# Christovis/astrild

Measured on AMD Instinct MI355X. Metric: particles/sec CIC+3D-FFT P(k) on 1024^3 grid, higher is better.
Workload: dtype f32

## Files before the change

### astrild_amd/csrc/mesh_paint_tiled.hip

```cpp
#include "ast_common.h"
#include "paint_tile_geom.h"
#include <algorithm>
#include <climits>
#include <cstdlib>
#include <mutex>
#include <type_traits>
#include <vector>

namespace {

using ast::Window;

using ast::TX;
using ast::TY;
using ast::TZ;
using ast::RingMap;
#ifndef PAINT_ABLATE
#define PAINT_ABLATE 0
#endif
constexpr int ablate = PAINT_ABLATE;

#ifdef PAINT_STAMPS
__device__ unsigned long long g_stamps[64 * 4096];
__device__ unsigned g_nstamp[64];
#define STAMP_DECL unsigned nst_ = 0
#define STAMP(id)                                                                                     \
    do {                                                                                              \
        if (threadIdx.x == 0 && blockIdx.x % 257 == 3 && blockIdx.x / 257 < 64 && nst_ < 4096)         \
            g_stamps[(blockIdx.x / 257) * 4096 + nst_++] = (__builtin_amdgcn_s_memtime() << 8) | (id); \
    } while (0)
#define STAMP_END                                                                                     \
    do {                                                                                              \
        if (threadIdx.x == 0 && blockIdx.x % 257 == 3 && blockIdx.x / 257 < 64) g_nstamp[blockIdx.x / 257] = nst_; \
    } while (0)
#else
#define STAMP_DECL
#define STAMP(id) do {} while (0)
#define STAMP_END do {} while (0)
#endif
#if defined(PAINT_STAMPS) && PAINT_STAMPS == 2
#define FSTAMP_DECL STAMP_DECL
#define FSTAMP(id) STAMP(id)
#define FSTAMP_END STAMP_END
#define DSTAMP_DECL
#define DSTAMP(id) do {} while (0)
#define DSTAMP_END do {} while (0)
#else
#define FSTAMP_DECL
#define FSTAMP(id) do {} while (0)
#define FSTAMP_END do {} while (0)
#define DSTAMP_DECL STAMP_DECL
#define DSTAMP(id) STAMP(id)
#define DSTAMP_END STAMP_END
#endif

struct TileGeom {
    int n, x_start, nx_alloc;
    int ntx, nty, ntz;
    double inv_dx;
    double shift;
    int off_lo, off_hi;
};

template <typename T> __device__ inline double grid_coord(T x, const TileGeom& g) { return __fma_rn((double)x, g.inv_dx, g.shift); }

template <typename T, int W, bool PLAINX>
__device__ inline uint32_t tile_of(T x, T y, T z, const TileGeom& g, uint32_t* __restrict__ col_flags) {
    const double sx = grid_coord(x, g), sy = grid_coord(y, g), sz = grid_coord(z, g);
    int cx = (int)floor(W == 2 ? sx : sx + 0.5);
    int cy = (int)floor(W == 2 ? sy : sy + 0.5);
    int cz = (int)floor(W == 2 ? sz : sz + 0.5);
    const bool far = max(max((unsigned)cx, (unsigned)cy), (unsigned)cz) >= (unsigned)g.n;
    if (far) {
        double f;
        cx = ast::locate<W>(sx, g.n, f);
        cy = ast::locate<W>(sy, g.n, f);
        cz = ast::locate<W>(sz, g.n, f);
    }
    unsigned bx = (unsigned)cx;
    if (!PLAINX) {
        int b = cx - g.x_start;
        if (b < 0) b += g.n;
        if (b >= g.nx_alloc) return 0xffffffffu;
        bx = (unsigned)b;
    }
    const uint32_t col = __umul24(bx / TX, (unsigned)g.nty) + (unsigned)cy / TY;
    if (far && col_flags && !(__hip_atomic_load(&col_flags[col], __ATOMIC_RELAXED, __HIP_MEMORY_SCOPE_AGENT) & 1u))
        atomicOr(&col_flags[col], 1u);
    return __umul24(col, (unsigned)g.ntz) + (unsigned)cz / TZ;
}

struct WaveRuns {
    bool head;
    int len;
    int head_lane;
};

__device__ inline WaveRuns wave_runs(uint32_t key, bool live, int lane) {
    WaveRuns r;
    const uint32_t prev = (uint32_t)__builtin_amdgcn_update_dpp((int)0xffffffffu, (int)key, 0x138, 0xf, 0xf, false);
    r.head = live && (lane == 0 || prev != key);
    const unsigned long long hmask = __ballot(r.head);
    const unsigned long long dmask = __ballot(!live);
    const unsigned long long above = ~((2ull << lane) - 1ull);
    const unsigned long long stop = (hmask | dmask) & above;
    const int end = stop ? __ffsll((long long)stop) - 1 : 64;
    r.len = end - lane;
    const unsigned long long at_or_below = hmask & ~above;
    r.head_lane = at_or_below ? 63 - __clzll((long long)at_or_below) : 0;
    return r;
}

constexpr int IDX_UNROLL = 4;
#ifndef AGG_TRIPS_N
#define AGG_TRIPS_N 4
#endif
constexpr int AGG_TRIPS = AGG_TRIPS_N;
constexpr int AGG_SLOTS = 256;
constexpr uint32_t SLOT_EMPTY = 0xffffffffu;
constexpr uint32_t CODE_DONE = 0xffffffffu;

template <int MODE>
__device__ __noinline__ void place_run_slow(uint32_t key, uint32_t p1, uint32_t len, const uint32_t* __restrict__ tile_off,
                                            uint32_t* __restrict__ tile_fill, uint32_t* __restrict__ index, uint32_t cap,
                                            uint32_t* __restrict__ ovf, unsigned long long* __restrict__ ovf_count) {
    const uint32_t b = atomicAdd(&tile_fill[key], len);
    for (uint32_t i = 0; i < len; ++i) {
        if (MODE == 1) index[(size_t)tile_off[key] + b + i] = p1 + i;
        else if (b + i < cap) index[(size_t)key * cap + b + i] = p1 + i;
        else ovf[atomicAdd(ovf_count, 1ull)] = p1 + i;
    }
}

template <typename T, int W, int MODE, bool PLAINX, int STRIDE = 3>
__global__ void __launch_bounds__(256)
tile_index_kernel(const T* __restrict__ pos, size_t np, TileGeom g, uint32_t* __restrict__ tile_count,
                  const uint32_t* __restrict__ tile_off, uint32_t* __restrict__ tile_fill,
                  uint32_t* __restrict__ index, uint32_t cap, uint32_t* __restrict__ ovf,
                  unsigned long long* __restrict__ ovf_count, uint32_t* __restrict__ col_flags,
                  unsigned long long* dropped, const unsigned long long* __restrict__ np_dev = nullptr,
                  unsigned long long np_min = 0) {
    constexpr bool FILL = MODE != 0;
    if (np_dev != nullptr) {
        const unsigned long long nd = *np_dev;
        if (nd < np_min || nd == 0) return;
        np = nd < np ? (size_t)nd : np;
    }
    __shared__ uint32_t skey[AGG_SLOTS], scnt[AGG_SLOTS], sroom[AGG_SLOTS];
    __shared__ unsigned long long sdst[AGG_SLOTS];
    __shared__ uint32_t codes[FILL ? AGG_TRIPS * IDX_UNROLL : 1][256];
    constexpr uint32_t MISS_CAP = FILL ? 512 : 1;
    __shared__ uint32_t smiss_key[MISS_CAP], smiss_p[MISS_CAP], smiss_len[MISS_CAP], smiss_n;
    FSTAMP_DECL;
    const int tid = threadIdx.x;
    const int lane = tid & 63;
    skey[tid] = SLOT_EMPTY;
    scnt[tid] = 0;
    if (tid == 0) smiss_n = 0;
    __syncthreads();
    const size_t per_trip = 256 * IDX_UNROLL;
    const size_t per_interval = per_trip * AGG_TRIPS;
    const size_t nintervals = (np + per_interval - 1) / per_interval;
    unsigned long long ndrop = 0;
    auto fetch = [&](size_t pbase, T (&x)[IDX_UNROLL], T (&y)[IDX_UNROLL], T (&z)[IDX_UNROLL]) {
#pragma unroll
        for (int u = 0; u < IDX_UNROLL; ++u) {
            const size_t p = min(pbase + (size_t)u * 256 + tid, np - 1);
            x[u] = pos[STRIDE * p + 0];
            y[u] = pos[STRIDE * p + 1];
            z[u] = pos[STRIDE * p + 2];
        }
    };
    auto place_run = [&](uint32_t key, uint32_t p1, uint32_t len) {
        place_run_slow<MODE>(key, p1, len, tile_off, tile_fill, index, cap, ovf, ovf_count);
    };
    static_assert(AGG_TRIPS % 2 == 0, "two register sets");
    T xa[IDX_UNROLL], ya[IDX_UNROLL], za[IDX_UNROLL], xb[IDX_UNROLL], yb[IDX_UNROLL], zb[IDX_UNROLL];
    if ((size_t)blockIdx.x < nintervals) fetch((size_t)blockIdx.x * per_interval, xa, ya, za);
    for (size_t interval = blockIdx.x; interval < nintervals; interval += gridDim.x) {
        const size_t p0 = interval * per_interval;
        const bool full = p0 + per_interval <= np;
        auto process = [&](int trip, const T (&x)[IDX_UNROLL], const T (&y)[IDX_UNROLL], const T (&z)[IDX_UNROLL]) {
#pragma unroll
            for (int u = 0; u < IDX_UNROLL; ++u) {
                const size_t p = p0 + (size_t)trip * per_trip + (size_t)u * 256 + tid;
                const bool valid = full || p < np;
                uint32_t key = tile_of<T, W, PLAINX>(x[u], y[u], z[u], g, MODE != 1 ? col_flags : nullptr);
                if (!valid) key = 0xffffffffu;
                const bool live = key != 0xffffffffu;
                if (!PLAINX && valid && !live) ++ndrop;
                const WaveRuns r = wave_runs(key, live, lane);
                bool parked = false;
                uint32_t val = 0;
                if (r.head) {
                    const uint32_t slot = (key * 2654435761u) >> 24;
                    const uint32_t old = atomicCAS(&skey[slot], SLOT_EMPTY, key);
                    if (old == SLOT_EMPTY || old == key) {
                        val = (slot << 16) | atomicAdd(&scnt[slot], (uint32_t)r.len);
                    } else if (MODE == 0) {
                        atomicAdd(&tile_count[key], (uint32_t)r.len);
                    } else {
                        parked = true;
                        const uint32_t mi = atomicAdd(&smiss_n, 1u);
                        if (mi < MISS_CAP) {
                            smiss_key[mi] = key;
                            smiss_p[mi] = (uint32_t)p;
                            smiss_len[mi] = (uint32_t)r.len;
                        } else {
                            place_run(key, (uint32_t)p, (uint32_t)r.len);
                        }
                    }
                }
                if (FILL) {
                    const uint32_t valb = __shfl(val, r.head_lane, 64) + (uint32_t)(lane - r.head_lane);
                    uint32_t code = live ? valb : CODE_DONE;
                    if (__any(parked)) {
                        if (__shfl((int)parked, r.head_lane, 64)) code = CODE_DONE;
                    }
                    codes[trip * IDX_UNROLL + u][tid] = code;
                }
            }
        };
#pragma unroll
        for (int trip = 0; trip < AGG_TRIPS; trip += 2) {
            FSTAMP(1);
            fetch(p0 + (size_t)(trip + 1) * per_trip, xb, yb, zb);
            process(trip, xa, ya, za);
            FSTAMP(2);
            fetch(trip + 2 < AGG_TRIPS ? p0 + (size_t)(trip + 2) * per_trip : (interval + gridDim.x) * per_interval, xa, ya, za);
            process(trip + 1, xb, yb, zb);
            FSTAMP(2);
        }
        __syncthreads();
        FSTAMP(3);
        if (skey[tid] != SLOT_EMPTY) {
            const uint32_t t = skey[tid], c = scnt[tid];
            if (MODE == 0) atomicAdd(&tile_count[t], c);
            else if (MODE == 1) { sdst[tid] = (unsigned long long)tile_off[t] + atomicAdd(&tile_fill[t], c); sroom[tid] = 0xffffffffu; }
            else {
                const uint32_t base = min(atomicAdd(&tile_fill[t], c), cap);
                sdst[tid] = (unsigned long long)t * cap + base;
                sroom[tid] = cap - base;
            }
        }
        if (FILL) {
            const uint32_t nm = min(smiss_n, MISS_CAP);
            for (uint32_t e = tid; e < nm; e += 256) {
                place_run(smiss_key[e], smiss_p[e], smiss_len[e]);
            }
        }
        FSTAMP(4);
        __syncthreads();
        FSTAMP(5);
        if (FILL) {
            if (tid == 0) smiss_n = 0;
#pragma unroll 4
            for (int j = 0; j < AGG_TRIPS * IDX_UNROLL; ++j) {
                const uint32_t c = codes[j][tid];
                if (c == CODE_DONE) continue;
                const uint32_t p = (uint32_t)(p0 + (size_t)j * 256 + tid);
                const uint32_t slot = c >> 16, at = c & 0xffffu;
                if (at < sroom[slot]) index[sdst[slot] + at] = p;
                else ovf[atomicAdd(ovf_count, 1ull)] = p;
            }
        }
        skey[tid] = SLOT_EMPTY;
        scnt[tid] = 0;
        FSTAMP(6);
        __syncthreads();
        FSTAMP(7);
    }
    FSTAMP_END;
    if (MODE != 1 && dropped && ndrop) atomicAdd(dropped, ndrop);
}

constexpr int MINPOP = 8;
#ifndef GROUP_ITERS_N
#define GROUP_ITERS_N 3
#endif
#ifndef GROUP_CAND
#define GROUP_CAND 16, 8, 24, 0
#endif
constexpr int GROUP_ITERS = GROUP_ITERS_N;
constexpr uint32_t LREC_CAP = 512;
struct GroupRec { uint32_t first, mask; };

template <typename T>
__device__ inline void store_stray(T* __restrict__ strays, size_t slot, T x, T y, T z, T m, bool has_mass) {
    typedef T vec4_t __attribute__((ext_vector_type(4)));
    struct Rec3 { T x, y, z; };
    if (has_mass) *reinterpret_cast<vec4_t*>(strays + 4 * slot) = vec4_t{x, y, z, m};
    else *reinterpret_cast<Rec3*>(strays + 3 * slot) = Rec3{x, y, z};
}

template <typename T>
__device__ __noinline__ void place_group_slow(uint32_t key, uint32_t a, uint32_t mask, const T* __restrict__ pos,
                                              const T* __restrict__ mass, unsigned long long* __restrict__ fill64,
                                              GroupRec* __restrict__ recs, uint32_t rcap, T* __restrict__ strays,
                                              uint32_t scap, uint32_t* __restrict__ ovf,
                                              unsigned long long* __restrict__ ovf_count) {
    if (mask) {
        const uint32_t r = (uint32_t)(atomicAdd(&fill64[key], 1ull << 32) >> 32);
        if (r < rcap) { recs[(size_t)key * rcap + r] = GroupRec{a, mask}; return; }
        for (uint32_t m = mask; m; m &= m - 1) ovf[atomicAdd(ovf_count, 1ull)] = a + (uint32_t)__ffs((int)m) - 1u;
    } else {
        const uint32_t sidx = (uint32_t)atomicAdd(&fill64[key], 1ull);
        if (sidx < scap) store_stray(strays, (size_t)key * scap + sidx, pos[3 * (size_t)a], pos[3 * (size_t)a + 1],
                                     pos[3 * (size_t)a + 2], mass ? mass[a] : (T)1, mass != nullptr);
        else ovf[atomicAdd(ovf_count, 1ull)] = a;
    }
}

constexpr uint32_t LST_CAP = 768;

__device__ __noinline__ void place_late_slow(uint32_t p, uint32_t* __restrict__ ovf, unsigned long long* __restrict__ ovf_count) {
    ovf[atomicAdd(ovf_count, 1ull)] = p;
}

template <typename T, int W, bool PLAINX>
__global__ void __launch_bounds__(256)
__attribute__((amdgpu_waves_per_eu(sizeof(T) == 4 ? 5 : 1, sizeof(T) == 4 ? 5 : 8)))
tile_group_kernel(const T* __restrict__ pos, const T* __restrict__ mass, size_t p_begin, size_t np, TileGeom g,
                  unsigned long long* __restrict__ fill64, GroupRec* __restrict__ recs, uint32_t rcap,
                  T* __restrict__ strays, uint32_t scap, uint32_t* __restrict__ ovf,
                  unsigned long long* __restrict__ ovf_count, uint32_t* __restrict__ col_flags,
                  unsigned long long* dropped, uint32_t closed_lo, uint32_t closed_n, uint32_t closed_mod = 0u,
                  uint32_t xcd_map = 0u) {
    __shared__ uint32_t skey[AGG_SLOTS], srun[AGG_SLOTS], sstray[AGG_SLOTS], sroom_run[AGG_SLOTS], sroom_stray[AGG_SLOTS];
    __shared__ unsigned long long sdst_run[AGG_SLOTS], sdst_stray[AGG_SLOTS];
    __shared__ uint32_t lrec_first[LREC_CAP], lrec_mask[LREC_CAP], lrec_key[LREC_CAP], lrec_n;
    __shared__ T lst_x[LST_CAP], lst_y[LST_CAP], lst_z[LST_CAP];
    __shared__ uint32_t lst_p[LST_CAP], lst_key[LST_CAP], lst_n;
    constexpr uint32_t DST_NONE = 0xffffffffu;
    FSTAMP_DECL;
    const int tid = threadIdx.x;
    const int lane = tid & 63;
    const int half = lane >> 5;
    skey[tid] = SLOT_EMPTY;
    srun[tid] = 0;
    sstray[tid] = 0;
    if (tid == 0) { lst_n = 0; lrec_n = 0; }
    __syncthreads();
    const size_t per_trip = 256 * IDX_UNROLL;
    const size_t per_interval = per_trip * AGG_TRIPS;
    const size_t nintervals = (np - p_begin + per_interval - 1) / per_interval;
    unsigned long long ndrop = 0;
    auto fetch = [&](size_t pbase, T (&x)[IDX_UNROLL], T (&y)[IDX_UNROLL], T (&z)[IDX_UNROLL]) {
        const size_t pb = min(pbase, np - 1);
        const T* __restrict__ bp = pos + 3 * pb;
        const uint32_t last = (uint32_t)min((size_t)(256 * IDX_UNROLL - 1), np - 1 - pb);
#pragma unroll
        for (int u = 0; u < IDX_UNROLL; ++u) {
            const uint32_t rel = 3u * min((uint32_t)(u * 256 + tid), last);
            x[u] = bp[rel + 0];
            y[u] = bp[rel + 1];
            z[u] = bp[rel + 2];
        }
    };
    auto slow = [&](uint32_t key, uint32_t a, uint32_t mask) {
        place_group_slow<T>(key, a, mask, pos, mass, fill64, recs, rcap, strays, scap, ovf, ovf_count);
    };
    auto slot_of = [&](uint32_t key) -> int {
        const uint32_t slot = (key * 2654435761u) >> 24;
        const uint32_t old = atomicCAS(&skey[slot], SLOT_EMPTY, key);
        return (old == SLOT_EMPTY || old == key) ? (int)slot : -1;
    };
    static_assert(AGG_TRIPS % 2 == 0, "two register sets");
    T xa[IDX_UNROLL], ya[IDX_UNROLL], za[IDX_UNROLL], xb[IDX_UNROLL], yb[IDX_UNROLL], zb[IDX_UNROLL];
    size_t vb = blockIdx.x;
    if (xcd_map && gridDim.x % 8u == 0u) vb = (size_t)(blockIdx.x % 8u) * (gridDim.x / 8u) + blockIdx.x / 8u;
    if (vb < nintervals) fetch(p_begin + vb * per_interval, xa, ya, za);
    for (size_t interval = vb; interval < nintervals; interval += gridDim.x) {
        const size_t p0 = p_begin + interval * per_interval;
        const bool full = p0 + per_interval <= np;
        const uint32_t p0_32 = (uint32_t)p0, left = (uint32_t)min(np - p0, per_interval);
        auto process = [&](int trip, const T (&x)[IDX_UNROLL], const T (&y)[IDX_UNROLL], const T (&z)[IDX_UNROLL]) {
#pragma unroll
            for (int u = 0; u < IDX_UNROLL; ++u) {
                const uint32_t prel = (uint32_t)(trip * (int)per_trip + u * 256 + tid);
                const uint32_t p = p0_32 + prel;
                const bool valid = full || prel < left;
                uint32_t key = tile_of<T, W, PLAINX>(x[u], y[u], z[u], g, col_flags);
                if (!valid) key = 0xffffffffu;
                if (!PLAINX && valid && key == 0xffffffffu) ++ndrop;
                uint32_t dkey = key - closed_lo;
                if (!PLAINX && closed_mod && key < closed_lo) dkey += closed_mod;
                if (dkey < closed_n && key != 0xffffffffu) {
                    if (!PLAINX && closed_mod) ++ndrop;
                    else place_late_slow(p, ovf, ovf_count);
                    key = 0xffffffffu;
                }
                const bool live = key != 0xffffffffu;
                bool pending = live, stray = false;
#pragma unroll
                for (int it = 0; it < GROUP_ITERS; ++it) {
                    constexpr int cand[4] = {GROUP_CAND};
                    const uint32_t k0 = (uint32_t)__builtin_amdgcn_readlane((int)key, cand[it]);
                    const uint32_t k1 = (uint32_t)__builtin_amdgcn_readlane((int)key, cand[it] + 32);
                    const bool match = pending && key == (half ? k1 : k0);
                    const unsigned long long mb = __ballot(match);
                    const uint32_t mlo = (uint32_t)mb, mhi = (uint32_t)(mb >> 32);
                    const uint32_t mm = half ? mhi : mlo;
                    const bool big = half ? __popc(mhi) >= MINPOP : __popc(mlo) >= MINPOP;
                    if (big) {
                        if (match && (lane & 31) == __ffs((int)mm) - 1) {
                            const uint32_t first = (uint32_t)p - (uint32_t)(lane & 31);
                            const uint32_t k = atomicAdd(&lrec_n, 1u);
                            if (k < LREC_CAP) {
                                lrec_first[k] = first;
                                lrec_mask[k] = mm;
                                lrec_key[k] = key;
                            } else {
                                slow(key, first, mm);
                            }
                        }
                    } else {
                        stray = stray || match;
                    }
                    pending = pending && !match;
                    const unsigned long long pend = __ballot(pending);
                    if (__popc((uint32_t)pend) < MINPOP && __popc((uint32_t)(pend >> 32)) < MINPOP) break;
                }
                stray = stray || pending;
                const unsigned long long sm = __ballot(stray);
                if (sm) {
                    const int lead = __ffsll((long long)sm) - 1;
                    uint32_t base = 0;
                    if (lane == lead) base = atomicAdd(&lst_n, (uint32_t)__popcll(sm));
                    base = (uint32_t)__builtin_amdgcn_readlane((int)base, lead);
                    if (stray) {
                        const uint32_t k = base + (uint32_t)__popcll(sm & ((1ull << lane) - 1ull));
                        if (k < LST_CAP) {
                            lst_x[k] = x[u];
                            lst_y[k] = y[u];
                            lst_z[k] = z[u];
                            lst_p[k] = (uint32_t)p;
                            lst_key[k] = key;
                        } else {
                            slow(key, (uint32_t)p, 0u);
                        }
                    }
                }
            }
        };
        FSTAMP(1);
#pragma unroll
        for (int trip = 0; trip < AGG_TRIPS; trip += 2) {
            fetch(p0 + (size_t)(trip + 1) * per_trip, xb, yb, zb);
            process(trip, xa, ya, za);
            fetch(trip + 2 < AGG_TRIPS ? p0 + (size_t)(trip + 2) * per_trip : p_begin + (interval + gridDim.x) * per_interval, xa, ya, za);
            process(trip + 1, xb, yb, zb);
        }
        FSTAMP(2);
        __syncthreads();
        FSTAMP(3);
        const uint32_t nr = min(lrec_n, LREC_CAP), ns = min(lst_n, LST_CAP);
        for (uint32_t k = tid; k < nr; k += 256) {
            const uint32_t key = lrec_key[k];
            const int slot = slot_of(key);
            if (slot < 0) { slow(key, lrec_first[k], lrec_mask[k]); lrec_key[k] = DST_NONE; }
            else lrec_key[k] = ((uint32_t)slot << 16) | atomicAdd(&srun[slot], 1u);
        }
        for (uint32_t k = tid; k < ns; k += 256) {
            const uint32_t key = lst_key[k];
            const int slot = slot_of(key);
            if (slot < 0) { slow(key, lst_p[k], 0u); lst_key[k] = DST_NONE; }
            else lst_key[k] = ((uint32_t)slot << 16) | atomicAdd(&sstray[slot], 1u);
        }
        FSTAMP(4);
        __syncthreads();
        FSTAMP(5);
        if (skey[tid] != SLOT_EMPTY) {
            const uint32_t t = skey[tid], cr = srun[tid], cs = sstray[tid];
            const unsigned long long old = atomicAdd(&fill64[t], ((unsigned long long)cr << 32) | cs);
            const uint32_t br = min((uint32_t)(old >> 32), rcap), bs = min((uint32_t)old, scap);
            sdst_run[tid] = (unsigned long long)t * rcap + br;
            sroom_run[tid] = rcap - br;
            sdst_stray[tid] = (unsigned long long)t * scap + bs;
            sroom_stray[tid] = scap - bs;
        }
        FSTAMP(6);
        __syncthreads();
        FSTAMP(7);
        for (uint32_t k = tid; k < nr; k += 256) {
            const uint32_t d = lrec_key[k];
            if (d == DST_NONE) continue;
            const uint32_t slot = d >> 16, at = d & 0xffffu;
            if (at < sroom_run[slot]) recs[sdst_run[slot] + at] = GroupRec{lrec_first[k], lrec_mask[k]};
            else for (uint32_t m = lrec_mask[k]; m; m &= m - 1) ovf[atomicAdd(ovf_count, 1ull)] = lrec_first[k] + (uint32_t)__ffs((int)m) - 1u;
        }
        for (uint32_t k = tid; k < ns; k += 256) {
            const uint32_t d = lst_key[k];
            if (d == DST_NONE) continue;
            const uint32_t slot = d >> 16, at = d & 0xffffu;
            if (at < sroom_stray[slot]) store_stray(strays, (size_t)(sdst_stray[slot] + at), lst_x[k], lst_y[k], lst_z[k],
                                                    mass ? mass[lst_p[k]] : (T)1, mass != nullptr);
            else ovf[atomicAdd(ovf_count, 1ull)] = lst_p[k];
        }
        FSTAMP(8);
        __syncthreads();
        skey[tid] = SLOT_EMPTY;
        srun[tid] = 0;
        sstray[tid] = 0;
        if (tid == 0) { lst_n = 0; lrec_n = 0; }
        __syncthreads();
        FSTAMP(9);
    }
    FSTAMP_END;
    if (dropped && ndrop) atomicAdd(dropped, ndrop);
}

#ifndef SCA_NT
#define SCA_NT 512
#endif
#ifndef SCB_NT
#define SCB_NT 512
#endif
constexpr int SC_PER_THREAD = 8;
constexpr int SCA_THREADS = SCA_NT, SCB_THREADS = SCB_NT;
constexpr uint32_t SC_BUCKETS_MAX = 1024, SC_TPB_MAX = 4 * SCB_NT;
constexpr uint32_t SC_GROUPS = 8;
#ifndef SCB_WGS
#define SCB_WGS 64
#endif
static_assert(SCB_WGS % SC_GROUPS == 0 && SCB_WGS >= SC_GROUPS, "level B: every (bucket, label) segment gets SCB_WGS / SC_GROUPS workgroups");

template <typename T, int NT> constexpr uint32_t sc_round() { return (sizeof(T) == 4 ? 4u : 2u) * (uint32_t)NT; }

template <int NT>
__device__ inline uint32_t block_exclusive_scan(const uint32_t* cnt, uint32_t* lstart, uint32_t table, uint32_t* wsum) {
    const int tid = threadIdx.x, lane = tid & 63, wave = tid >> 6;
    const uint32_t K = table > 2u * NT ? 4u : 2u, i0 = K * tid;
    uint32_t v[4], own = 0;
#pragma unroll
    for (uint32_t k = 0; k < 4; ++k) { v[k] = (k < K && i0 + k < table) ? cnt[i0 + k] : 0u; own += v[k]; }
    uint32_t inc = own;
#pragma unroll
    for (int o = 1; o < 64; o <<= 1) { const uint32_t t = __shfl_up(inc, o, 64); if (lane >= o) inc += t; }
    if (lane == 63) wsum[wave] = inc;
    __syncthreads();
    uint32_t woff = 0, total = 0;
    for (int k = 0; k < NT / 64; ++k) { if (k < wave) woff += wsum[k]; total += wsum[k]; }
    uint32_t ex = woff + inc - own;
#pragma unroll
    for (uint32_t k = 0; k < 4; ++k) { if (k < K && i0 + k < table) lstart[i0 + k] = ex; ex += v[k]; }
    __syncthreads();
    return total;
}

template <typename T, int SW, int NT>
__device__ inline void staged_store(const T (&rx)[SC_PER_THREAD], const T (&ry)[SC_PER_THREAD], const T (&rz)[SC_PER_THREAD],
                                    const T (&rm)[SC_PER_THREAD], const uint32_t (&where)[SC_PER_THREAD],
                                    const uint32_t* lstart, const unsigned long long* base, const uint32_t* room,
                                    uint32_t total, T* __restrict__ out, T* stage ,
                                    unsigned long long* sidx ) {
    typedef T vec4_t __attribute__((ext_vector_type(4)));
    struct Rec3 { T x, y, z; };
    constexpr uint32_t ROUND = sc_round<T, NT>();
    for (uint32_t q0 = 0; q0 < total; q0 += ROUND) {
#pragma unroll
        for (int u = 0; u < SC_PER_THREAD; ++u) {
            if (where[u] == 0xffffffffu) continue;
            const uint32_t e = where[u] >> 16, r = where[u] & 0xffffu;
            const uint32_t sl = lstart[e] + r - q0;
            if (sl < ROUND) {
                if (SW == 4) reinterpret_cast<vec4_t*>(stage)[sl] = vec4_t{rx[u], ry[u], rz[u], rm[u]};
                else reinterpret_cast<Rec3*>(stage)[sl] = Rec3{rx[u], ry[u], rz[u]};
                sidx[sl] = (room == nullptr || r < room[e]) ? base[e] + r : ~0ull;
            }
        }
        __syncthreads();
        const uint32_t here = min(ROUND, total - q0);
        for (uint32_t i = threadIdx.x; i < here; i += NT) {
            const unsigned long long d = sidx[i];
            if (d == ~0ull) continue;
            if (SW == 4) *reinterpret_cast<vec4_t*>(out + 4 * (size_t)d) = reinterpret_cast<const vec4_t*>(stage)[i];
            else *reinterpret_cast<Rec3*>(out + 3 * (size_t)d) = reinterpret_cast<const Rec3*>(stage)[i];
        }
        __syncthreads();
    }
}

__device__ inline unsigned long long wave_append(unsigned long long* __restrict__ counter, bool want) {
    const unsigned long long m = __ballot(want);
    if (m == 0ull) return 0ull;
    const int lane = (int)(threadIdx.x & 63u), leader = __ffsll((long long)m) - 1;
    unsigned long long base = 0ull;
    if (lane == leader) base = atomicAdd(counter, (unsigned long long)__popcll(m));
    base = __shfl(base, leader, 64);
    return base + (unsigned long long)__popcll(m & ((1ull << lane) - 1ull));
}

template <typename T, int W, bool PLAINX, int SW>
__global__ void __launch_bounds__(SCA_THREADS)
scatter_level_a_kernel(const T* __restrict__ pos, const T* __restrict__ mass, size_t np, TileGeom g, uint32_t tpb, uint32_t nb,
                       unsigned long long* __restrict__ cursor, T* __restrict__ staging, uint32_t cap_bg,
                       uint32_t* __restrict__ col_flags, T* __restrict__ late_list, unsigned long long late_cap,
                       unsigned long long* __restrict__ late, unsigned long long* dropped) {
    __shared__ uint32_t cnt[SC_BUCKETS_MAX], lstart[SC_BUCKETS_MAX], room[SC_BUCKETS_MAX], wsum[16];
    __shared__ unsigned long long base[SC_BUCKETS_MAX];
    extern __shared__ unsigned long long dyn[];
    T* stage = reinterpret_cast<T*>(dyn);
    constexpr int NT = SCA_THREADS, SC_CHUNK = NT * SC_PER_THREAD;
    unsigned long long* sidx = dyn + sc_round<T, NT>() * SW * sizeof(T) / sizeof(unsigned long long);
    typedef T vec4_t __attribute__((ext_vector_type(4)));
    const int tid = threadIdx.x;
    for (uint32_t b = tid; b < nb; b += NT) cnt[b] = 0;
    __syncthreads();
    const size_t p0 = (size_t)blockIdx.x * SC_CHUNK;
    T x[SC_PER_THREAD], y[SC_PER_THREAD], z[SC_PER_THREAD], m[SC_PER_THREAD];
    uint32_t where[SC_PER_THREAD];
    const T* __restrict__ bp = pos + 3 * p0;
    const uint32_t last = (uint32_t)min(np - 1 - p0, (size_t)(SC_CHUNK - 1));
#pragma unroll
    for (int u = 0; u < SC_PER_THREAD; ++u) {
        const uint32_t rel = min((uint32_t)(u * NT + tid), last);
        x[u] = bp[3 * rel];
        y[u] = bp[3 * rel + 1];
        z[u] = bp[3 * rel + 2];
        m[u] = SW == 4 && mass ? mass[p0 + rel] : (T)1;
    }
    unsigned long long ndrop = 0;
#pragma unroll
    for (int u = 0; u < SC_PER_THREAD; ++u) {
        where[u] = 0xffffffffu;
        if ((uint32_t)(u * NT + tid) <= last) {
            const uint32_t key = tile_of<T, W, PLAINX>(x[u], y[u], z[u], g, col_flags);
            if (key != 0xffffffffu) {
                const uint32_t b = key / tpb;
                where[u] = (b << 16) | atomicAdd(&cnt[b], 1u);
            } else {
                ++ndrop;
            }
        }
    }
    __syncthreads();
    const uint32_t grp = blockIdx.x % SC_GROUPS;
    __shared__ int any_full;
    if (tid == 0) any_full = 0;
    __syncthreads();
    for (uint32_t b = tid; b < nb; b += NT) {
        if (!cnt[b]) continue;
        const unsigned long long old = atomicAdd(&cursor[grp * nb + b], (unsigned long long)cnt[b]);
        const uint32_t bs = (uint32_t)min(old, (unsigned long long)cap_bg);
        base[b] = ((unsigned long long)b * SC_GROUPS + grp) * cap_bg + bs;
        room[b] = cap_bg - bs;
        if (cnt[b] > cap_bg - bs) any_full = 1;
    }
    const uint32_t total = block_exclusive_scan<NT>(cnt, lstart, nb, wsum);
    const bool full = any_full != 0;
    if (full) {
#pragma unroll
        for (int u = 0; u < SC_PER_THREAD; ++u) {
            const bool over = where[u] != 0xffffffffu && (where[u] & 0xffffu) >= room[where[u] >> 16];
            const unsigned long long k = wave_append(late, over);
            if (over) {
                if (k < late_cap) reinterpret_cast<vec4_t*>(late_list)[k] = vec4_t{x[u], y[u], z[u], m[u]};
// ... 1084 lines not shown
        AST_PROF("paint_tiled.overflow", s);
        const unsigned long long lds_min = hooks.late_lds_set ? hooks.late_lds_min : sizeof(T) == 4 ? 1ull : 262144ull;
        late_global(1024, 0, g.nx_alloc, lds_min);
        if (lds_min != ~0ull && late_cap() > 0) {
            const T* list = (const T*)w.ovf;
            const unsigned gl = interval_grid((size_t)late_cap(), 4096);
            index_pass<0, 4>(list, (size_t)late_cap(), gl, w.tile_count, w.tile_off, w.tile_fill, w.late_index, 0, nullptr, nullptr, nullptr, w.late, lds_min);
            tile_scan();
            index_pass<1, 4>(list, (size_t)late_cap(), gl, w.tile_count, w.tile_off, w.tile_fill, w.late_index, 0, nullptr, nullptr, nullptr, w.late, lds_min);
            tile_deposit_kernel<T, W, 4><<<ntiles < 8192u ? ntiles : 8192u, 256, 0, s>>>(list, nullptr, g, scale, w.late_index, w.tile_off,
                                                                                       w.tile_count, 0, grid, dropped, ntiles);
        }
        return AST_OK;
    }
    int accumulate_path() {
        {
            AST_PROF("paint_tiled.fill", s);
            index_pass<2>(pos, np, interval_grid(np), nullptr, nullptr, w.tile_fill, w.index, w.cap, w.ovf, w.ovf_count, dropped);
        }
        deposit(nullptr, w.tile_fill, w.cap);
        overflow(1024, 0, g.nx_alloc);
        return AST_OK;
    }
    int grouped_path() {
        group(0, np, 0u, 0u);
        deposit(nullptr, nullptr, 0);
        overflow(1024, 0, g.nx_alloc);
        return AST_OK;
    }
    int enqueue_chunks(SidePipe* sp, hipEvent_t& last_walk) {
        const int K = plan.chunks;
        const int m0 = g.nx_alloc == g.n ? 1 : 0;
        const uint32_t rs = (uint32_t)(g.nty * g.ntz);
        int prev = m0, nev = 0;
        hipEvent_t walk_done[2] = {nullptr, nullptr};
        for (int k = 0; k < K; ++k) {
            const auto part = part_bounds(k, 1, K);
            if (sp && walk_done[1]) AST_CHECK_HIP(hipStreamWaitEvent(s, walk_done[1], 0));
            if (part.second > part.first) group(part.first, part.second, (uint32_t)m0 * rs, (uint32_t)(prev - m0) * rs);
            const int covered = (int)((long long)(k + 1) * g.nx_alloc / K) - plan.margin_planes;
            const int r = k + 1 == K ? g.ntx : std::max(prev, std::min(g.ntx, covered / TX));
            if (r > prev || k + 1 == K) {
                const int rows = r - prev + (k + 1 == K ? m0 : 0);
                hipStream_t ws = s;
                if (sp) {
                    AST_CHECK_HIP(hipEventRecord(sp->ev[nev], s));
                    AST_CHECK_HIP(hipStreamWaitEvent(sp->side, sp->ev[nev], 0));
                    ++nev;
                    ws = sp->side;
                }
                if (rows > 0) walk(nullptr, nullptr, prev * g.nty, (unsigned)(rows * g.nty), ws);
                if (sp) {
                    AST_CHECK_HIP(hipEventRecord(sp->ev[nev], sp->side));
                    walk_done[1] = walk_done[0];
                    last_walk = walk_done[0] = sp->ev[nev];
                    ++nev;
                }
                prev = r;
            }
        }
        return AST_OK;
    }
    int xsorted_path() {
        {
            const bool two_streams = plan.streams > 1;
            SidePipe* sp = two_streams ? side_pipe(2 * g.ntx + 4) : nullptr;
            if (two_streams && !sp) { ast::set_error("ast_paint_tiled: no side stream"); return AST_ERR_HIP; }
            AST_PROF("paint_tiled.pipeline", s);
            std::unique_lock<std::mutex> pipe_lock;
            if (sp) pipe_lock = std::unique_lock<std::mutex>(sp->run);
            hipEvent_t last_walk = nullptr;
            const int rc = enqueue_chunks(sp, last_walk);
            if (rc != AST_OK && sp) (void)hipStreamSynchronize(sp->side);
            if (rc != AST_OK) return rc;
            if (last_walk) AST_CHECK_HIP(hipStreamWaitEvent(s, last_walk, 0));
            seams_and_fold();
        }
        overflow(1024, 0, g.nx_alloc);
        return AST_OK;
    }

    int stage(const StageSel& sel) {
        if (two_pass || !overwrite || (flags & (AST_PAINT_DEFER_FOLD | AST_PAINT_XSORTED))) {
            ast::set_error("ast_paint_tiled_stage: needs AST_PAINT_OVERWRITE without TWO_PASS / DEFER_FOLD / XSORTED");
            return AST_ERR_ARG;
        }
        if (sel.stage == AST_PAINT_STAGE_RESET) return AST_OK;
        if (sel.stage == AST_PAINT_STAGE_GROUP) {
            if (w.tpb) { const int rc = scatter_levels(); if (rc != AST_OK) return rc; }
            else group(0, np, 0u, 0u);
        } else if (sel.stage == AST_PAINT_STAGE_GROUP_PART) {
            const int k = sel.row0, K = sel.nrows & 0xffff, span = (sel.nrows >> 16) + 1;
            if (w.tpb || plainx || K < 1 || k < 0 || span < 1 || k + span > K || sel.closed_nrows < 0 || sel.closed_nrows > g.ntx ||
                sel.closed_row0 < 0 || sel.closed_row0 >= g.ntx) {
                ast::set_error("ast_paint_tiled_stage: GROUP_PART needs a slab buffer (not the scattered path), 0 <= part, part + span <= parts and closed rows inside the buffer");
                return AST_ERR_ARG;
            }
            const auto part = part_bounds(k, span, K);
            const uint32_t rs = (uint32_t)(g.nty * g.ntz);
            if (part.second > part.first) group(part.first, part.second, (uint32_t)sel.closed_row0 * rs, (uint32_t)sel.closed_nrows * rs, ntiles);
        } else {
            if (sel.row0 < 0 || sel.nrows < 1 || sel.row0 + sel.nrows > g.ntx) {
                ast::set_error("ast_paint_tiled_stage: tile rows [%d, %d) outside [0, %d)", sel.row0, sel.row0 + sel.nrows, g.ntx);
                return AST_ERR_ARG;
            }
            const int col0 = sel.row0 * g.nty;
            const unsigned ncol = (unsigned)(sel.nrows * g.nty);
            if (sel.stage == AST_PAINT_STAGE_WALK) {
                walk(nullptr, nullptr, col0, ncol, s);
                seams(col0, ncol);
            } else if (sel.stage == AST_PAINT_STAGE_FOLD || sel.stage == AST_PAINT_STAGE_LATE) {
                if (sel.stage == AST_PAINT_STAGE_FOLD) fold(col0, ncol);
                const int x_lo = sel.row0 * TX, x_hi = std::min(g.nx_alloc, (sel.row0 + sel.nrows) * TX);
                if (w.tpb) {
                    AST_PROF("paint_tiled.overflow", s);
                    late_global(128, x_lo, x_hi);
                } else {
                    overflow(128, x_lo, x_hi);
                }
            } else {
                ast::set_error("ast_paint_tiled_stage: unknown stage %d", sel.stage);
                return AST_ERR_ARG;
            }
        }
        AST_CHECK_LAUNCH();
        return AST_OK;
    }

    int run(const StageSel& sel) {
        if (sel.stage == AST_PAINT_STAGE_ALL || sel.stage == AST_PAINT_STAGE_GROUP || sel.stage == AST_PAINT_STAGE_RESET)
            AST_CHECK_HIP(hipMemsetAsync(w.ovf_count, 0, (size_t)((char*)w.tile_off - (char*)w.ovf_count), s));
        if (sel.stage != AST_PAINT_STAGE_ALL) return stage(sel);
        const int rc = two_pass ? two_pass_path() : !overwrite ? accumulate_path() : w.tpb ? scattered_path()
                     : plan.chunks > 1 ? xsorted_path() : grouped_path();
        if (rc != AST_OK) return rc;
        AST_CHECK_LAUNCH();
        return AST_OK;
    }
};

}

#ifdef PAINT_STAMPS
extern "C" int ast_debug_stamps(unsigned long long* stamps_host, unsigned* counts_host) {
    AST_CHECK_HIP(hipDeviceSynchronize());
    AST_CHECK_HIP(hipMemcpyFromSymbol(stamps_host, HIP_SYMBOL(g_stamps), sizeof(unsigned long long) * 64 * 4096));
    AST_CHECK_HIP(hipMemcpyFromSymbol(counts_host, HIP_SYMBOL(g_nstamp), sizeof(unsigned) * 64));
    unsigned zero[64] = {0};
    AST_CHECK_HIP(hipMemcpyToSymbol(HIP_SYMBOL(g_nstamp), zero, sizeof(zero)));
    return AST_OK;
}
#endif

extern "C" size_t ast_paint_scatter_late_capacity(int dtype, size_t np) {
    if (dtype != AST_F32 && dtype != AST_F64) return 0;
    return (size_t)late_capacity(np, dtype == AST_F32 ? 4 : 8);
}

extern "C" size_t ast_paint_tiled_workspace_bytes(int window, int dtype, size_t np, int nmesh, int nx_alloc, int flags) {
    TileGeom g;
    if (nmesh <= 0 || nx_alloc <= 0 || !tiled_geometry(nmesh, nx_alloc, g)) return 0;
    return paint_layout(nullptr, window, dtype == AST_F32 ? 4 : 8, np, g, flags, read_test_hooks()).bytes;
}

extern "C" int ast_paint_tiled_halo(void* workspace, int window, int dtype, size_t np, int nmesh, int nx_alloc, int flags,
                                    void** rec_out) {
    AST_CHECK_ARG(workspace && rec_out && (flags & AST_PAINT_OVERWRITE));
    AST_CHECK_ARG(window == AST_WIN_CIC || window == AST_WIN_TSC);
    TileGeom g;
    AST_CHECK_ARG(nmesh > 0 && nx_alloc > 0 && tiled_geometry(nmesh, nx_alloc, g));
    *rec_out = paint_layout(workspace, window, dtype == AST_F32 ? 4 : 8, np, g, flags, read_test_hooks()).rec;
    return AST_OK;
}

__global__ void __launch_bounds__(256)
list_stats_kernel(const unsigned long long* __restrict__ fill64, uint32_t ntiles, uint32_t rcap, uint32_t scap,
                  const unsigned long long* __restrict__ ovf_count, unsigned long long* out) {
    unsigned long long nr = 0, ns = 0, smax = 0;
    for (uint32_t t = blockIdx.x * blockDim.x + threadIdx.x; t < ntiles; t += gridDim.x * blockDim.x) {
        const unsigned long long f = fill64[t];
        nr += min((uint32_t)(f >> 32), rcap);
        ns += min((uint32_t)f, scap);
        smax = max(smax, (unsigned long long)(uint32_t)f);
    }
    atomicAdd(&out[0], nr);
    atomicAdd(&out[1], ns);
    atomicMax(&out[3], smax);
    if (blockIdx.x == 0 && threadIdx.x == 0) out[2] = *ovf_count;
}

extern "C" int ast_paint_tiled_list_stats(void* workspace, int window, int dtype, size_t np, int nmesh, int nx_alloc,
                                          int flags, unsigned long long* out, void* stream) {
    AST_CHECK_ARG(workspace && out && (flags & AST_PAINT_OVERWRITE) && !(flags & AST_PAINT_TWO_PASS));
    TileGeom g;
    AST_CHECK_ARG(nmesh > 0 && nx_alloc > 0 && tiled_geometry(nmesh, nx_alloc, g));
    const Workspace w = paint_layout(workspace, window, dtype == AST_F32 ? 4 : 8, np, g, flags, read_test_hooks());
    hipStream_t s = ast::as_stream(stream);
    AST_CHECK_HIP(hipMemsetAsync(out, 0, 4 * sizeof(unsigned long long), s));
    list_stats_kernel<<<256, 256, 0, s>>>(w.fill64, w.ntiles, w.rcap, w.scap, w.tpb ? w.late : w.ovf_count, out);
    AST_CHECK_LAUNCH();
    return AST_OK;
}

template <typename T>
__global__ void __launch_bounds__(64)
order_probe_kernel(const T* __restrict__ pos, size_t np, int n, double inv_dx, double shift, int windows,
                   unsigned* __restrict__ groupable) {
    const size_t w = blockIdx.x;
    size_t start = (w * (np - 32) / (size_t)(windows - 1)) / 32 * 32;
    if (start > np - 32) start = np - 32;
    const int lane = threadIdx.x;
    unsigned long long key = ~0ull;
    if (lane < 32) {
        const T* p = pos + 3 * (start + lane);
        long long c[3];
#pragma unroll
        for (int a = 0; a < 3; ++a) {
            const double sc = floor(__fma_rn((double)p[a], inv_dx, shift));
            long long ci = (long long)fmod(sc, (double)n);
            if (ci < 0) ci += n;
            c[a] = ci;
        }
        key = ((unsigned long long)(c[0] / ast::TX) * (unsigned long long)n + (unsigned long long)(c[1] / ast::TY)) * (unsigned long long)n +
              (unsigned long long)(c[2] / ast::TZ);
    }
    const unsigned long long k15 = __shfl(key, 15, 64);
    const unsigned long long same = __ballot(lane < 32 && key == k15);
    if (lane == 0 && __popcll(same) >= 8) atomicAdd(groupable, 1u);
}

extern "C" int ast_paint_order_probe(const void* pos, int dtype, size_t np, int nmesh, double boxsize, double shift_cells,
                                     int windows, unsigned* groupable, void* stream) {
    AST_CHECK_ARG(pos != nullptr && groupable != nullptr && (dtype == AST_F32 || dtype == AST_F64));
    AST_CHECK_ARG(np >= 32 && nmesh > 0 && boxsize > 0.0 && windows >= 2 && windows <= 65536);
    hipStream_t s = ast::as_stream(stream);
    AST_CHECK_HIP(hipMemsetAsync(groupable, 0, sizeof(unsigned), s));
    const double inv_dx = (double)nmesh / boxsize;
    if (dtype == AST_F32) order_probe_kernel<float><<<windows, 64, 0, s>>>((const float*)pos, np, nmesh, inv_dx, shift_cells, windows, groupable);
    else order_probe_kernel<double><<<windows, 64, 0, s>>>((const double*)pos, np, nmesh, inv_dx, shift_cells, windows, groupable);
    AST_CHECK_LAUNCH();
    return AST_OK;
}

__device__ inline uint64_t probe_mix(uint64_t z) {
    z += 0x9e3779b97f4a7c15ull;
    z = (z ^ (z >> 30)) * 0xbf58476d1ce4e5b9ull;
    z = (z ^ (z >> 27)) * 0x94d049bb133111ebull;
    return z ^ (z >> 31);
}
template <typename T>
__global__ void __launch_bounds__(256)
occupancy_sample_kernel(const T* __restrict__ pos, size_t np, int n, double inv_dx, double shift, size_t samples,
                        unsigned* __restrict__ counts) {
    const size_t i = (size_t)blockIdx.x * 256 + threadIdx.x;
    if (i >= samples) return;
    const size_t lo = (size_t)(((unsigned __int128)i * np) / samples), hi = (size_t)(((unsigned __int128)(i + 1) * np) / samples);
    const size_t j = lo + (hi > lo ? probe_mix(i) % (hi - lo) : 0);
    const T* p = pos + 3 * j;
    unsigned c[3];
#pragma unroll
    for (int a = 0; a < 3; ++a) {
        const double sc = floor(__fma_rn((double)p[a], inv_dx, shift));
        long long ci = (long long)fmod(sc, (double)n);
        if (ci < 0) ci += n;
        c[a] = (unsigned)ci;
    }
    const unsigned tile = ((c[0] / ast::TX) * (unsigned)(n / ast::TY) + c[1] / ast::TY) * (unsigned)(n / ast::TZ) + c[2] / ast::TZ;
    atomicAdd(&counts[tile], 1u);
}
__global__ void __launch_bounds__(256)
occupancy_excess_kernel(const unsigned* __restrict__ counts, unsigned ntiles, double per_sample, double cap,
                        unsigned long long* __restrict__ out) {
    __shared__ double ex[256];
    __shared__ double mx[256];
    double e = 0.0, m = 0.0;
    for (unsigned t = blockIdx.x * 256 + threadIdx.x; t < ntiles; t += gridDim.x * 256) {
        const double occ = (double)counts[t] * per_sample;
        if (occ > cap) e += occ - cap;
        m = occ > m ? occ : m;
    }
    ex[threadIdx.x] = e;
    mx[threadIdx.x] = m;
    __syncthreads();
    for (int st = 128; st > 0; st >>= 1) {
        if ((int)threadIdx.x < st) {
            ex[threadIdx.x] += ex[threadIdx.x + st];
            mx[threadIdx.x] = mx[threadIdx.x + st] > mx[threadIdx.x] ? mx[threadIdx.x + st] : mx[threadIdx.x];
        }
        __syncthreads();
    }
    if (threadIdx.x == 0) {
        atomicAdd(&out[0], (unsigned long long)(ex[0] + 0.5));
        atomicMax(&out[1], (unsigned long long)(mx[0] + 0.5));
    }
}

extern "C" size_t ast_paint_occupancy_probe_bytes(int nmesh) {
    if (nmesh <= 0 || nmesh % TY || nmesh % TZ || nmesh % TX) return 0;
    return (size_t)(nmesh / TX) * (nmesh / TY) * (nmesh / TZ) * sizeof(unsigned);
}

extern "C" int ast_paint_occupancy_probe(const void* pos, int dtype, size_t np, int nmesh, double boxsize, double shift_cells,
                                         size_t samples, void* counts, size_t counts_bytes, unsigned long long* out, void* stream) {
    AST_CHECK_ARG(pos != nullptr && counts != nullptr && out != nullptr && (dtype == AST_F32 || dtype == AST_F64));
    AST_CHECK_ARG(np >= 1 && boxsize > 0.0 && samples >= 1 && samples <= np && samples < (1ull << 40));
    const size_t need = ast_paint_occupancy_probe_bytes(nmesh);
// ... 104 lines not shown
```

Baseline: 86.09 billion.

## Use per-wave LDS record/stray lists and scalar ballot grouping in tile_group_kernel

Splits the shared group-record and stray lists into per-wave slices whose counters live in registers. This replaces the LDS atomicAdd on lrec_n/lst_n with a wave-local running count, and the per-wave counts are published before the barrier and turned into prefix offsets. It also adds a scalar grouping path that computes candidate masks for both half-waves with ballots in uniform registers, instead of per-lane match and popcount logic. The trade-offs are fixed per-wave capacities, so strays can overflow to the slow global path sooner if one wave is skewed, and an extra index remap in the flush loops.

```diff
diff --git a/astrild_amd/csrc/mesh_paint_tiled.hip b/astrild_amd/csrc/mesh_paint_tiled.hip
--- a/astrild_amd/csrc/mesh_paint_tiled.hip
+++ b/astrild_amd/csrc/mesh_paint_tiled.hip
@@ -1,5 +1,6 @@
 #include "ast_common.h"
 #include "paint_tile_geom.h"
+#include "paint_group_lists.h"
 #include <algorithm>
 #include <climits>
 #include <cstdlib>
@@ -282,7 +283,28 @@
 #define GROUP_CAND 16, 8, 24, 0
 #endif
 constexpr int GROUP_ITERS = GROUP_ITERS_N;
+#ifndef GROUP_SCALAR_N
+#define GROUP_SCALAR_N 1
+#endif
+#ifndef GROUP_WAVE_LISTS_N
+#define GROUP_WAVE_LISTS_N 1
+#endif
+#if GROUP_WAVE_LISTS_N
+constexpr uint32_t WREC_CAP = ast::wave_record_capacity(AGG_TRIPS * IDX_UNROLL, GROUP_ITERS);
+#ifndef WST_CAP_N
+#define WST_CAP_N 200
+#define WST_CAP_IS_DEFAULT 1
+#endif
+constexpr uint32_t WST_CAP = WST_CAP_N;
+constexpr uint32_t LREC_CAP = 4 * WREC_CAP, LST_CAP = 4 * WST_CAP;
+#ifdef WST_CAP_IS_DEFAULT
+static_assert(3 * LREC_CAP + 5 * LST_CAP <= 3 * 512 + 5 * 768 && 3 * LREC_CAP + 8 * LST_CAP <= 3 * 512 + 8 * 768,
+              "the lists (3 words per record, 5 or 8 per stray) must not grow: 31 KB of LDS are five workgroups per CU at float32");
+#endif
+#else
 constexpr uint32_t LREC_CAP = 512;
+constexpr uint32_t LST_CAP = 768;
+#endif
 struct GroupRec { uint32_t first, mask; };
 
 template <typename T>
@@ -311,7 +333,6 @@
     }
 }
 
-constexpr uint32_t LST_CAP = 768;
 
 __device__ __noinline__ void place_late_slow(uint32_t p, uint32_t* __restrict__ ovf, unsigned long long* __restrict__ ovf_count) {
     ovf[atomicAdd(ovf_count, 1ull)] = p;
@@ -328,18 +349,28 @@
                   uint32_t xcd_map = 0u) {
     __shared__ uint32_t skey[AGG_SLOTS], srun[AGG_SLOTS], sstray[AGG_SLOTS], sroom_run[AGG_SLOTS], sroom_stray[AGG_SLOTS];
     __shared__ unsigned long long sdst_run[AGG_SLOTS], sdst_stray[AGG_SLOTS];
-    __shared__ uint32_t lrec_first[LREC_CAP], lrec_mask[LREC_CAP], lrec_key[LREC_CAP], lrec_n;
+    __shared__ uint32_t lrec_first[LREC_CAP], lrec_mask[LREC_CAP], lrec_key[LREC_CAP];
     __shared__ T lst_x[LST_CAP], lst_y[LST_CAP], lst_z[LST_CAP];
-    __shared__ uint32_t lst_p[LST_CAP], lst_key[LST_CAP], lst_n;
+    __shared__ uint32_t lst_p[LST_CAP], lst_key[LST_CAP];
+#if GROUP_WAVE_LISTS_N
+    __shared__ uint32_t wave_nrec[4], wave_nst[4];
+#else
+    __shared__ uint32_t lrec_n, lst_n;
+#endif
     constexpr uint32_t DST_NONE = 0xffffffffu;
     FSTAMP_DECL;
     const int tid = threadIdx.x;
     const int lane = tid & 63;
     const int half = lane >> 5;
+#if GROUP_SCALAR_N || GROUP_WAVE_LISTS_N
+    const uint32_t wave = (uint32_t)__builtin_amdgcn_readfirstlane(tid >> 6);
+#endif
     skey[tid] = SLOT_EMPTY;
     srun[tid] = 0;
     sstray[tid] = 0;
+#if !GROUP_WAVE_LISTS_N
     if (tid == 0) { lst_n = 0; lrec_n = 0; }
+#endif
     __syncthreads();
     const size_t per_trip = 256 * IDX_UNROLL;
     const size_t per_interval = per_trip * AGG_TRIPS;
@@ -374,6 +405,9 @@
         const size_t p0 = p_begin + interval * per_interval;
         const bool full = p0 + per_interval <= np;
         const uint32_t p0_32 = (uint32_t)p0, left = (uint32_t)min(np - p0, per_interval);
+#if GROUP_WAVE_LISTS_N
+        uint32_t wrec_n = 0, wst_n = 0;
+#endif
         auto process = [&](int trip, const T (&x)[IDX_UNROLL], const T (&y)[IDX_UNROLL], const T (&z)[IDX_UNROLL]) {
 #pragma unroll
             for (int u = 0; u < IDX_UNROLL; ++u) {
@@ -391,6 +425,83 @@
                     key = 0xffffffffu;
                 }
                 const bool live = key != 0xffffffffu;
+#if GROUP_SCALAR_N
+                const unsigned long long lv = __ballot(live);
+                uint32_t pend_lo = (uint32_t)lv, pend_hi = (uint32_t)(lv >> 32), str_lo = 0, str_hi = 0;
+                const uint32_t first_lo = p0_32 + (uint32_t)(trip * (int)per_trip + u * 256) + wave * 64u;
+#pragma unroll
+                for (int it = 0; it < GROUP_ITERS; ++it) {
+                    constexpr int cand[4] = {GROUP_CAND};
+                    const uint32_t k0 = (uint32_t)__builtin_amdgcn_readlane((int)key, cand[it]);
+                    const uint32_t k1 = (uint32_t)__builtin_amdgcn_readlane((int)key, cand[it] + 32);
+                    const uint32_t m_lo = (uint32_t)__ballot(key == k0) & pend_lo;
+                    const uint32_t m_hi = (uint32_t)(__ballot(key == k1) >> 32) & pend_hi;
+                    const uint32_t big_lo = ((uint32_t)__popc(m_lo) + (32u - MINPOP)) >> 5;
+                    const uint32_t big_hi = ((uint32_t)__popc(m_hi) + (32u - MINPOP)) >> 5;
+                    if (big_lo | big_hi) {
+                        const uint32_t nrec = big_lo + big_hi;
+#if GROUP_WAVE_LISTS_N
+                        const uint32_t base = wave * WREC_CAP + wrec_n;
+                        wrec_n += nrec;
+#else
+                        uint32_t base = 0;
+                        if (lane == 0) base = atomicAdd(&lrec_n, nrec);
+                        base = (uint32_t)__builtin_amdgcn_readfirstlane((int)base);
+#endif
+                        const unsigned long long writers = (unsigned long long)big_lo | ((unsigned long long)big_hi << 32);
+                        if (__builtin_amdgcn_inverse_ballot_w64(writers)) {
+                            const uint32_t k = base + (half ? big_lo : 0u);
+                            const uint32_t rfirst = first_lo + (half ? 32u : 0u), rmask = half ? m_hi : m_lo, rkey = half ? k1 : k0;
+#if GROUP_WAVE_LISTS_N
+                            {
+#else
+                            if (k >= LREC_CAP) {
+                                slow(rkey, rfirst, rmask);
+                            } else {
+#endif
+                                lrec_first[k] = rfirst;
+                                lrec_mask[k] = rmask;
+                                lrec_key[k] = rkey;
+                            }
+                        }
+                    }
+                    str_lo |= m_lo & (big_lo - 1u);
+                    str_hi |= m_hi & (big_hi - 1u);
+                    pend_lo &= ~m_lo;
+                    pend_hi &= ~m_hi;
+                    if (__popc(pend_lo) < MINPOP && __popc(pend_hi) < MINPOP) break;
+                }
+                str_lo |= pend_lo;
+                str_hi |= pend_hi;
+                const unsigned long long sm = (unsigned long long)str_lo | ((unsigned long long)str_hi << 32);
+                if (sm) {
+                    const uint32_t cnt = (uint32_t)__popc(str_lo) + (uint32_t)__popc(str_hi);
+#if GROUP_WAVE_LISTS_N
+                    const uint32_t at = wst_n;
+                    wst_n += cnt;
+                    constexpr uint32_t room = WST_CAP;
+                    const uint32_t slice = wave * WST_CAP;
+#else
+                    uint32_t at = 0;
+                    if (lane == 0) at = atomicAdd(&lst_n, cnt);
+                    at = (uint32_t)__builtin_amdgcn_readfirstlane((int)at);
+                    constexpr uint32_t room = LST_CAP, slice = 0;
+#endif
+                    if (__builtin_amdgcn_inverse_ballot_w64(sm)) {
+                        const uint32_t i = at + __builtin_amdgcn_mbcnt_hi(str_hi, __builtin_amdgcn_mbcnt_lo(str_lo, 0u));
+                        if (i < room) {
+                            const uint32_t k = slice + i;
+                            lst_x[k] = x[u];
+                            lst_y[k] = y[u];
+                            lst_z[k] = z[u];
+                            lst_p[k] = (uint32_t)p;
+                            lst_key[k] = key;
+                        } else {
+                            slow(key, (uint32_t)p, 0u);
+                        }
+                    }
+                }
+#else
                 bool pending = live, stray = false;
 #pragma unroll
                 for (int it = 0; it < GROUP_ITERS; ++it) {
@@ -402,6 +513,18 @@
                     const uint32_t mlo = (uint32_t)mb, mhi = (uint32_t)(mb >> 32);
                     const uint32_t mm = half ? mhi : mlo;
                     const bool big = half ? __popc(mhi) >= MINPOP : __popc(mlo) >= MINPOP;
+#if GROUP_WAVE_LISTS_N
+                    const bool writer = big && match && (lane & 31) == __ffs((int)mm) - 1;
+                    const unsigned long long wb = __ballot(writer);
+                    if (writer) {
+                        const uint32_t k = wave * WREC_CAP + wrec_n + (half && (uint32_t)wb ? 1u : 0u);
+                        lrec_first[k] = (uint32_t)p - (uint32_t)(lane & 31);
+                        lrec_mask[k] = mm;
+                        lrec_key[k] = key;
+                    }
+                    wrec_n += (uint32_t)__popcll(wb);
+                    stray = stray || (match && !big);
+#else
                     if (big) {
                         if (match && (lane & 31) == __ffs((int)mm) - 1) {
                             const uint32_t first = (uint32_t)p - (uint32_t)(lane & 31);
@@ -417,6 +540,7 @@
                     } else {
                         stray = stray || match;
                     }
+#endif
                     pending = pending && !match;
                     const unsigned long long pend = __ballot(pending);
                     if (__popc((uint32_t)pend) < MINPOP && __popc((uint32_t)(pend >> 32)) < MINPOP) break;
@@ -424,13 +548,22 @@
                 stray = stray || pending;
                 const unsigned long long sm = __ballot(stray);
                 if (sm) {
+#if GROUP_WAVE_LISTS_N
+                    const uint32_t base = wst_n;
+                    wst_n += (uint32_t)__popcll(sm);
+                    constexpr uint32_t room = WST_CAP;
+                    const uint32_t slice = wave * WST_CAP;
+#else
                     const int lead = __ffsll((long long)sm) - 1;
                     uint32_t base = 0;
                     if (lane == lead) base = atomicAdd(&lst_n, (uint32_t)__popcll(sm));
                     base = (uint32_t)__builtin_amdgcn_readlane((int)base, lead);
+                    constexpr uint32_t room = LST_CAP, slice = 0;
+#endif
                     if (stray) {
-                        const uint32_t k = base + (uint32_t)__popcll(sm & ((1ull << lane) - 1ull));
-                        if (k < LST_CAP) {
+                        const uint32_t i = base + (uint32_t)__popcll(sm & ((1ull << lane) - 1ull));
+                        const uint32_t k = slice + i;
+                        if (i < room) {
                             lst_x[k] = x[u];
                             lst_y[k] = y[u];
                             lst_z[k] = z[u];
@@ -441,6 +574,7 @@
                         }
                     }
                 }
+#endif
             }
         };
         FSTAMP(1);
@@ -452,16 +586,33 @@
             process(trip + 1, xb, yb, zb);
         }
         FSTAMP(2);
+#if GROUP_WAVE_LISTS_N
+        if (lane == 0) {
+            wave_nrec[wave] = wrec_n;
+            wave_nst[wave] = min(wst_n, WST_CAP);
+        }
+#endif
         __syncthreads();
         FSTAMP(3);
+#if GROUP_WAVE_LISTS_N
+        const uint32_t r1 = wave_nrec[0], r2 = r1 + wave_nrec[1], r3 = r2 + wave_nrec[2], nr = r3 + wave_nrec[3];
+        const uint32_t s1 = wave_nst[0], s2 = s1 + wave_nst[1], s3 = s2 + wave_nst[2], ns = s3 + wave_nst[3];
+        auto rec_at = [&](uint32_t e) { return ast::slice_entry(e, r1, r2, r3, WREC_CAP); };
+        auto stray_at = [&](uint32_t e) { return ast::slice_entry(e, s1, s2, s3, WST_CAP); };
+#else
         const uint32_t nr = min(lrec_n, LREC_CAP), ns = min(lst_n, LST_CAP);
-        for (uint32_t k = tid; k < nr; k += 256) {
+        auto rec_at = [](uint32_t e) { return e; };
+        auto stray_at = [](uint32_t e) { return e; };
+#endif
+        for (uint32_t e = tid; e < nr; e += 256) {
+            const uint32_t k = rec_at(e);
             const uint32_t key = lrec_key[k];
             const int slot = slot_of(key);
             if (slot < 0) { slow(key, lrec_first[k], lrec_mask[k]); lrec_key[k] = DST_NONE; }
             else lrec_key[k] = ((uint32_t)slot << 16) | atomicAdd(&srun[slot], 1u);
         }
-        for (uint32_t k = tid; k < ns; k += 256) {
+        for (uint32_t e = tid; e < ns; e += 256) {
+            const uint32_t k = stray_at(e);
             const uint32_t key = lst_key[k];
             const int slot = slot_of(key);
             if (slot < 0) { slow(key, lst_p[k], 0u); lst_key[k] = DST_NONE; }
@@ -482,14 +633,16 @@
         FSTAMP(6);
         __syncthreads();
         FSTAMP(7);
-        for (uint32_t k = tid; k < nr; k += 256) {
+        for (uint32_t e = tid; e < nr; e += 256) {
+            const uint32_t k = rec_at(e);
             const uint32_t d = lrec_key[k];
             if (d == DST_NONE) continue;
             const uint32_t slot = d >> 16, at = d & 0xffffu;
             if (at < sroom_run[slot]) recs[sdst_run[slot] + at] = GroupRec{lrec_first[k], lrec_mask[k]};
             else for (uint32_t m = lrec_mask[k]; m; m &= m - 1) ovf[atomicAdd(ovf_count, 1ull)] = lrec_first[k] + (uint32_t)__ffs((int)m) - 1u;
         }
-        for (uint32_t k = tid; k < ns; k += 256) {
+        for (uint32_t e = tid; e < ns; e += 256) {
+            const uint32_t k = stray_at(e);
             const uint32_t d = lst_key[k];
             if (d == DST_NONE) continue;
             const uint32_t slot = d >> 16, at = d & 0xffffu;
@@ -502,7 +655,9 @@
         skey[tid] = SLOT_EMPTY;
         srun[tid] = 0;
         sstray[tid] = 0;
+#if !GROUP_WAVE_LISTS_N
         if (tid == 0) { lst_n = 0; lrec_n = 0; }
+#endif
         __syncthreads();
         FSTAMP(9);
     }
@@ -1893,6 +2048,7 @@
 }
 #endif
 
+
 extern "C" size_t ast_paint_scatter_late_capacity(int dtype, size_t np) {
     if (dtype != AST_F32 && dtype != AST_F64) return 0;
     return (size_t)late_capacity(np, dtype == AST_F32 ? 4 : 8);
diff --git a/astrild_amd/csrc/paint_group_lists.h b/astrild_amd/csrc/paint_group_lists.h
--- /dev/null
+++ b/astrild_amd/csrc/paint_group_lists.h
@@ -0,0 +1,20 @@
+#pragma once
+#include <cstdint>
+
+#if defined(__HIPCC__) || defined(__CUDACC__)
+#define AST_GROUP_HD __host__ __device__
+#else
+#define AST_GROUP_HD
+#endif
+
+namespace ast {
+
+constexpr int GROUP_WAVES = 4;
+
+AST_GROUP_HD constexpr uint32_t wave_record_capacity(int slots, int iters) { return (uint32_t)(slots * 2 * iters); }
+
+AST_GROUP_HD inline uint32_t slice_entry(uint32_t e, uint32_t e1, uint32_t e2, uint32_t e3, uint32_t cap) {
+    return e + (e >= e3 ? 3u * cap - e3 : e >= e2 ? 2u * cap - e2 : e >= e1 ? cap - e1 : 0u);
+}
+
+}
```

After: 87.40 billion, median of 6. 1.02x the previous value.
